# facebookresearch/KeypointNeRF

Measured on AMD Instinct MI355X. Metric: rendered rays/sec (64 coarse + 64 fine samples/ray), higher is better.
Workload: dtype f32 (dominant kernel: every fp32 operand as two fp16 pieces (22 bits, the residual formed exactly), three fp16-MFMA products per term set (hh hl lh: all terms above 2^-24 relative), fp32 accumulation; everything else fp32)

## Files before the change

include/kpnerf.h:

```cpp
#ifndef KPNERF_H
#define KPNERF_H

#include <stddef.h>
#include <stdint.h>

#ifdef __cplusplus
extern "C" {
#endif

#define KPN_ABI_VERSION 5
#define KPN_N_KPT 24
#define KPN_MAX_VIEWS 16

enum { KPN_OK = 0, KPN_EINVAL = -1, KPN_ELAUNCH = -2, KPN_EWORKSPACE = -3 };

int kpn_abi_version(void);
const char* kpn_last_error(void);
int kpn_is_device_build(void);

size_t kpn_plain_weight_floats(void);
size_t kpn_packed_weight_floats(void);
int kpn_pack_weights(const float* plain_host, float* packed_host);
int kpn_pack_weights_device(const float* plain_dev, float* packed_dev, void* stream);

typedef struct kpn_scene_desc {
    int32_t n_views;
    int32_t src_h, src_w;
    int32_t geo0_h, geo0_w;
    int32_t geo1_h, geo1_w;
    int32_t tex_h, tex_w;
    int32_t disable_fg_mask;
    float znear, zfar;
    float nml_scale;
    float sigma;
    const float* KRT;
    const float* extrin;
    const float* kpt3d;
    const float* img;
    const uint8_t* fg_mask;
    const float* geo0;
    const float* geo1;
    const float* tex;
} kpn_scene_desc;

size_t kpn_scene_workspace_bytes(const kpn_scene_desc* desc);
int kpn_scene_prepare(const kpn_scene_desc* desc, void* scene_ws, void* stream);


int kpn_ray_bbox_intersection(const float* bounds, const float* orig, const float* direct, int64_t n_rays,
                              float* near_out, float* far_out, uint8_t* hit_out, void* stream);

int kpn_make_rays(const float* K, const float* RT, float znear, float zfar, const float* bounds, int32_t x0,
                  int32_t y0, int32_t step, int32_t nx, int32_t ny, float* dirs, float* cam_pos, float* near_out,
                  float* far_out, void* stream);

int kpn_importance_sample(const float* contrib, const float* z, const float* u, int64_t n_rays, int32_t d_minus_2,
                          int32_t n_samples, float* samples_out, void* stream);

int kpn_rgba2out(const float* rgba, const float* z, int64_t n_rays, int32_t n_samples, float* color, float* depth,
                 float* alpha, float* contrib, float* sdf, void* stream);

int kpn_rgba2out_backward(const float* rgba, const float* z, int64_t n_rays, int32_t n_samples, const float* d_color,
                          const float* d_depth, const float* d_alpha, const float* d_sdf, float* d_rgba, void* stream);

size_t kpn_geo_rows_backward_workspace_bytes(int64_t n_points, int32_t n_views);
int kpn_geo_rows_backward(const kpn_scene_desc* desc, const void* scene_ws, const float* packed_weights, int64_t n_points,
                          const float* pts, uint32_t keep_mask, const float* d_x, float* d_plain, float* d_geo0,
                          float* d_geo1, void* workspace, size_t workspace_bytes, void* stream);

size_t kpn_query_backward_geometry_workspace_bytes(int64_t n_points, int32_t n_views);
int kpn_query_backward_geometry(const kpn_scene_desc* desc, const void* scene_ws, const float* packed_weights,
                                int64_t n_points, const float* pts, int32_t mode, uint32_t keep_mask, const float* noise,
                                float noise_std, const float* d_out, float* d_plain, float* d_geo0, float* d_geo1,
                                void* workspace, size_t workspace_bytes, void* stream);

size_t kpn_query_backward_workspace_bytes(int64_t n_points, int32_t n_views);
int kpn_query_backward(const kpn_scene_desc* desc, const void* scene_ws, const float* packed_weights, int64_t n_points,
                       const float* pts, const float* view, int32_t mode, uint32_t keep_mask, const float* noise,
                       float noise_std, const float* d_out, float* d_plain, float* d_geo0, float* d_geo1, float* d_tex,
                       void* workspace, size_t workspace_bytes, void* stream);

int kpn_set_geo_rows_mode(int32_t mode);
int kpn_get_geo_rows_mode(void);
int kpn_set_fuse_mode(int32_t mode);
int kpn_get_fuse_mode(void);
int kpn_set_density_first(int32_t mode);
int kpn_get_density_first(void);
int kpn_density_first_passes(int64_t* density_first, int64_t* fused, int32_t reset);
int kpn_density_stats(void* stream, int64_t* listed, int64_t* live, int32_t reset);
int kpn_packed_f16_range_check(const float* packed_weights_dev, void* stream, int32_t* beyond);
// ... 134 lines not shown
```

keypointnerf_amd/csrc/api_render.hip:

```cpp
namespace {
struct RenderLayout { size_t cam_pos, dirs, nearv, farv, zc, zf, zn, src, rgba, rgba_c, rgba_n, contrib, color, depth, alpha, sdf, query, total; int64_t chunk; };
int64_t pick_chunk(const kpn_scene_desc* d, const kpn_render_args* a) {
    const int64_t R = (int64_t)a->nx * a->ny;
    int64_t c = a->chunk_rays;
    if (c <= 0) {
        const int64_t cmax = 262144;
        const int64_t npass = (R + cmax - 1) / cmax;
        c = ((R + npass - 1) / npass + 63) / 64 * 64;
    }
    return c < R ? c : R;
}
RenderLayout render_layout(const kpn_scene_desc* d, const kpn_render_args* a) {
    RenderLayout L;
    const int64_t R = (int64_t)a->nx * a->ny;
    const int64_t C = pick_chunk(d, a);
    const int64_t Sfull = a->n_coarse + (a->fine ? a->n_fine : 0);
    Carver c;
    L.chunk = C;
    L.cam_pos = c.take(64);
    L.dirs = c.take((size_t)R * 3 * 4);
    L.nearv = c.take((size_t)R * 4);
    L.farv = c.take((size_t)R * 4);
    L.zc = c.take((size_t)C * a->n_coarse * 4);
    L.zf = c.take((size_t)C * Sfull * 4);
// ... 38 lines not shown
}

__global__ void k_store_planar(int64_t r0, int64_t n, int64_t R, int C, const float* __restrict__ src, float* __restrict__ dst) {
    const int64_t i = (int64_t)blockIdx.x * blockDim.x + threadIdx.x;
    if (i >= n * C) return;
    const int64_t r = i / C;
    const int c = (int)(i - r * C);
    dst[(int64_t)c * R + r0 + r] = src[i];
}
__global__ void k_load_planar(int64_t r0, int64_t n, int64_t R, int C, const float* __restrict__ src, float* __restrict__ dst) {
    const int64_t i = (int64_t)blockIdx.x * blockDim.x + threadIdx.x;
    if (i >= n * C) return;
    const int64_t r = i / C;
    const int c = (int)(i - r * C);
    dst[i] = src ? src[(int64_t)c * R + r0 + r] : 0.0f;
}
struct PlanarChunk {
    void* stream; int64_t r0, n, R;
    void store(float* dst, const float* src, int C) const {
        if (dst) KPN_LAUNCH(k_store_planar, grid1d(n * C, 256), dim3(256), stream, r0, n, R, C, src, dst);
    }
    void load(float* dst, const float* src, int C) const {
        KPN_LAUNCH(k_load_planar, grid1d(n * C, 256), dim3(256), stream, r0, n, R, C, src, dst);
    }
};

extern "C" size_t kpn_render_workspace_bytes(const kpn_scene_desc* d, const kpn_render_args* a) {
    if (check_desc(d) != KPN_OK || check_render(a) != KPN_OK) return 0;
    return render_layout(d, a).total;
}

static void launch_fine_samples(void* stream, int64_t n, int Sc, int Sf, const float* zc, const float* contrib,
                                const float* u, float* zf, float* znew, int16_t* src) {
    const dim3 grid((unsigned)(n + 3 < 4 * 8192 ? (n + 3) / 4 : 8192));
    if (Sc <= 64 && Sf <= 64)
        KPN_LAUNCH(k_fine_samples_w<true>, grid, dim3(256), stream, n, Sc, Sf, zc, contrib, u, zf, znew, src);
    else
        KPN_LAUNCH(k_fine_samples_w<false>, grid, dim3(256), stream, n, Sc, Sf, zc, contrib, u, zf, znew, src);
}

static int render_impl(const kpn_scene_desc* d, const void* scene_ws, const float* wp, const kpn_render_args* a,
                       const kpn_train_args* t, void* ws, size_t ws_bytes, void* stream) {
    if (int e = check_desc(d)) return e;
    if (int e = check_render(a)) return e;
    KPN_REQUIRE(scene_ws && wp && ws, "null pointer");
    if (t) if (int e = check_train(d, a, t, false)) return e;
    const RenderLayout L = render_layout(d, a);
    if (ws_bytes < L.total) return fail(KPN_EWORKSPACE, "render workspace too small");
    char* base = static_cast<char*>(ws);
    auto F = [&](size_t off) { return reinterpret_cast<float*>(base + off); };
    kpn_scene_dev sc = scene_dev(d, scene_ws);
    const int64_t R = (int64_t)a->nx * a->ny;
    const int Sc = a->n_coarse, Sf = a->fine ? a->n_fine : 0, Sfull = Sc + Sf;
    KPN_LAUNCH(k_make_rays, grid1d(R, 256), dim3(256), stream, a->K, a->RT, a->znear, a->zfar, a->bounds, (int)a->x0, (int)a->y0,
               (int)a->step, (int)(a->step_y > 0 ? a->step_y : a->step), (int)a->nx, (int)a->ny, t ? (const int*)t->pix : (const int*)nullptr, F(L.dirs), F(L.cam_pos),
               F(L.nearv), F(L.farv));
    for (int64_t r0 = 0; r0 < R; r0 += L.chunk) {
        const int64_t n = (R - r0) < L.chunk ? (R - r0) : L.chunk;
        const float* dirs = F(L.dirs) + r0 * 3;
        const PlanarChunk pl{stream, r0, n, R};
        KPN_LAUNCH(k_coarse_z, grid1d(n * Sc, 256), dim3(256), stream, n, Sc, (const float*)(F(L.nearv) + r0),
                   (const float*)(F(L.farv) + r0), t ? t->u_coarse + r0 * Sc : (const float*)nullptr, F(L.zc));
        kpn_points ps{nullptr, nullptr, F(L.cam_pos), dirs, F(L.zc), Sc,
                      (t && t->rand_noise_std != 0.0f) ? t->noise_coarse + r0 * Sc : nullptr, t ? t->rand_noise_std : 0.0f};
        sc.keep = t ? t->keep_coarse : 0xFFFFFFFFu;
        const char* nr = getenv("KPN_NO_COARSE_REUSE");
        const bool no_reuse = nr && atoi(nr);
        const bool reuse = (t == nullptr) && a->fine && !no_reuse;
        float* rgba_coarse = reuse ? F(L.rgba_c) : F(L.rgba);
        const int allow_pool = t == nullptr;
        if (int e = run_field(sc, ps, wp, n * Sc, 1, rgba_coarse, nullptr, base + L.query, stream, 1, 0, allow_pool, a->rows_kernel, a->fuse_kernel)) return e;
// ... 232 lines not shown
```

keypointnerf_amd/csrc/api_scene.hip:

```cpp
namespace {
struct SceneLayout { size_t table, rgbm, geo0, geo1, tex, flags, total; };
SceneLayout scene_layout(const kpn_scene_desc* d) {
    SceneLayout L;
    Carver c;
    L.table = c.take((size_t)d->n_views * KPN_TBL_STRIDE, 64);
    L.rgbm = c.take((size_t)d->n_views * d->src_h * d->src_w * 4, 64);
    L.geo0 = c.take((size_t)d->n_views * d->geo0_h * d->geo0_w * 64, 64);
    L.geo1 = c.take((size_t)d->n_views * d->geo1_h * d->geo1_w * 8, 64);
    L.tex = c.take((size_t)d->n_views * d->tex_h * d->tex_w * 8, 64);
    L.flags = c.take((size_t)KPN_SCENE_FLAG_FLOATS, 64);
    L.total = c.o;
    return L;
}
int check_desc(const kpn_scene_desc* d) {
    KPN_REQUIRE(d != nullptr, "scene desc is null");
    KPN_REQUIRE(d->n_views >= 1 && d->n_views <= KPN_MAX_VIEWS, "n_views out of range");
    KPN_REQUIRE(d->src_h > 1 && d->src_w > 1 && d->geo0_h > 1 && d->geo0_w > 1 && d->geo1_h > 1 && d->geo1_w > 1 &&
                d->tex_h > 1 && d->tex_w > 1, "map sizes must be > 1");
    KPN_REQUIRE(d->zfar > d->znear && d->nml_scale > 0.0f && d->sigma > 0.0f, "bad scalar parameters");
    KPN_REQUIRE(d->KRT && d->extrin && d->kpt3d && d->img && d->geo0 && d->geo1 && d->tex, "null scene tensor");
    KPN_REQUIRE(d->disable_fg_mask || d->fg_mask, "fg_mask is null");
    return KPN_OK;
}
kpn_scene_dev scene_dev(const kpn_scene_desc* d, const void* ws) {
    const SceneLayout L = scene_layout(d);
    const float* base = static_cast<const float*>(ws);
    kpn_scene_dev s;
    s.V = d->n_views; s.H = d->src_h; s.W = d->src_w;
    s.g0h = d->geo0_h; s.g0w = d->geo0_w; s.g1h = d->geo1_h; s.g1w = d->geo1_w; s.th = d->tex_h; s.tw = d->tex_w;
    s.disable_fg_mask = d->disable_fg_mask;
    s.znear = d->znear; s.zfar = d->zfar; s.nml_scale = d->nml_scale;
    s.two_sigma2 = (float)(2.0 * ((double)d->sigma * (double)d->sigma));
    s.keep = 0xFFFFFFFFu;
    s.table = base + L.table; s.rgbm = base + L.rgbm; s.geo0 = base + L.geo0; s.geo1 = base + L.geo1; s.tex = base + L.tex;
    s.flags = base + L.flags;
    return s;
}
}

extern "C" size_t kpn_scene_workspace_bytes(const kpn_scene_desc* d) {
    if (check_desc(d) != KPN_OK) return 0;
    return scene_layout(d).total * sizeof(float);
}

extern "C" int kpn_scene_prepare(const kpn_scene_desc* d, void* scene_ws, void* stream) {
    if (int e = check_desc(d)) return e;
    KPN_REQUIRE(scene_ws != nullptr, "scene workspace is null");
    const SceneLayout L = scene_layout(d);
    float* base = static_cast<float*>(scene_ws);
    const int V = d->n_views;
    float* flags = base + L.flags;
    KPN_LAUNCH(k_scene_table, dim3(1), dim3(64), stream, V, d->KRT, d->extrin, d->kpt3d, base + L.table, flags);
    const int64_t HW = (int64_t)d->src_h * d->src_w;
    KPN_LAUNCH(k_pack_rgbm, grid1d(V * HW, 256), dim3(256), stream, (int64_t)(V * HW), HW, d->img,
               d->disable_fg_mask ? (const uint8_t*)nullptr : d->fg_mask, base + L.rgbm, flags);
    const int64_t hw0 = (int64_t)d->geo0_h * d->geo0_w, hw1 = (int64_t)d->geo1_h * d->geo1_w, hwt = (int64_t)d->tex_h * d->tex_w;
    KPN_LAUNCH(k_nchw_to_nhwc, grid1d(V * hw0 * 64, 256), dim3(256), stream, (int64_t)(V * hw0 * 64), 64, hw0, d->geo0, base + L.geo0, flags);
    KPN_LAUNCH(k_nchw_to_nhwc, grid1d(V * hw1 * 8, 256), dim3(256), stream, (int64_t)(V * hw1 * 8), 8, hw1, d->geo1, base + L.geo1, flags);
    KPN_LAUNCH(k_nchw_to_nhwc, grid1d(V * hwt * 8, 256), dim3(256), stream, (int64_t)(V * hwt * 8), 8, hwt, d->tex, base + L.tex, flags);
    return check_launch("kpn_scene_prepare");
}

extern "C" int kpn_ray_bbox_intersection(const float* bounds, const float* orig, const float* direct, int64_t R,
                                         float* near_o, float* far_o, uint8_t* hit_o, void* stream) {
    KPN_REQUIRE(bounds && orig && direct && near_o && far_o && hit_o, "null pointer");
    KPN_REQUIRE(R >= 0, "negative ray count");
    if (R == 0) return KPN_OK;
    KPN_LAUNCH(k_ray_bbox, grid1d(R, 256), dim3(256), stream, R, bounds, orig, direct, near_o, far_o, hit_o);
    return check_launch("kpn_ray_bbox_intersection");
}

extern "C" int kpn_make_rays(const float* K, const float* RT, float znear, float zfar, const float* bounds, int32_t x0,
                             int32_t y0, int32_t step, int32_t nx, int32_t ny, float* dirs, float* cam_pos,
                             float* near_o, float* far_o, void* stream) {
    KPN_REQUIRE(K && RT && bounds && dirs && cam_pos && near_o && far_o, "null pointer");
    KPN_REQUIRE(nx > 0 && ny > 0 && step > 0, "bad pixel grid");
    KPN_LAUNCH(k_make_rays, grid1d((int64_t)nx * ny, 256), dim3(256), stream, K, RT, znear, zfar, bounds, (int)x0, (int)y0,
               (int)step, (int)step, (int)nx, (int)ny, (const int*)nullptr, dirs, cam_pos, near_o, far_o);
    return check_launch("kpn_make_rays");
}

extern "C" int kpn_importance_sample(const float* contrib, const float* z, const float* u, int64_t R, int32_t Dm2,
                                     int32_t n, float* out, void* stream) {
    KPN_REQUIRE(contrib && z && out, "null pointer");
    KPN_REQUIRE(Dm2 >= 1 && Dm2 + 1 <= KPN_IS_MAXD, "bin count out of range (<= 128)");
    KPN_REQUIRE(n >= 1 && R >= 0, "bad sizes");
    if (R == 0) return KPN_OK;
    KPN_LAUNCH(k_importance, grid1d(R, 64), dim3(64), stream, R, (int)Dm2, (int)n, contrib, z, u, out);
    return check_launch("kpn_importance_sample");
}

static void launch_rgba2out(void* stream, int64_t R, int S, const float* rgba, const float* z, float* color, float* depth,
// ... 39 lines not shown
```

keypointnerf_amd/csrc/ray_kernels.hip:

```cpp
#include "kpn_device.h"

__device__ __forceinline__ void kpn_note_absmax(float* __restrict__ flags, float a) {
    int u = __float_as_int(a) & 0x7fffffff;
#pragma unroll
    for (int o = 32; o > 0; o >>= 1) { const int w = __shfl_xor(u, o); u = w > u ? w : u; }
    int* f = reinterpret_cast<int*>(flags);
    if ((threadIdx.x & 63) == 0 && u > *reinterpret_cast<volatile int*>(f)) atomicMax(f, u);
}
__device__ __forceinline__ float kpn_absmax2(float a, float b) {
    const int x = __float_as_int(a) & 0x7fffffff, y = __float_as_int(b) & 0x7fffffff;
    return __int_as_float(x > y ? x : y);
}

__global__ void k_scene_table(int V, const float* __restrict__ KRT, const float* __restrict__ extrin,
                              const float* __restrict__ kpt3d, float* __restrict__ table, float* __restrict__ flags) {
    const int v = blockIdx.x * blockDim.x + threadIdx.x;
    if (v < KPN_SCENE_FLAG_FLOATS) flags[v] = 0.0f;
    if (v >= V) return;
    float* tb = table + (size_t)v * KPN_TBL_STRIDE;
    const float* M = KRT + v * 16;
    const float* E = extrin + v * 16;
    for (int i = 0; i < 12; ++i) { tb[KPN_TBL_KRT + i] = M[i]; tb[KPN_TBL_EXT + i] = E[i]; }
    double a[4][8];
    for (int i = 0; i < 4; ++i)
        for (int j = 0; j < 4; ++j) { a[i][j] = (double)M[i * 4 + j]; a[i][4 + j] = (i == j) ? 1.0 : 0.0; }
    for (int c = 0; c < 4; ++c) {
        int p = c;
        for (int r = c + 1; r < 4; ++r) if (fabs(a[r][c]) > fabs(a[p][c])) p = r;
        if (p != c) for (int j = 0; j < 8; ++j) { double t = a[c][j]; a[c][j] = a[p][j]; a[p][j] = t; }
        const double d = a[c][c];
        for (int j = 0; j < 8; ++j) a[c][j] /= d;
        for (int r = 0; r < 4; ++r) if (r != c) {
            const double f = a[r][c];
            for (int j = 0; j < 8; ++j) a[r][j] -= f * a[c][j];
        }
    }
    for (int i = 0; i < 3; ++i) tb[KPN_TBL_CPOS + i] = (float)a[i][7];
    tb[KPN_TBL_CPOS + 3] = 0.0f;
    for (int k = 0; k < KPN_NKPT; ++k)
        for (int i = 0; i < 3; ++i)
            tb[KPN_TBL_KCAM + k * 3 + i] =
                KADD(kpn_dot3(kpt3d[k * 3 + 0], kpt3d[k * 3 + 1], kpt3d[k * 3 + 2], E[i * 4 + 0], E[i * 4 + 1], E[i * 4 + 2]),
                     E[i * 4 + 3]);
    for (int i = KPN_TBL_KCAM + KPN_NKPT * 3; i < KPN_TBL_STRIDE; ++i) tb[i] = 0.0f;
}

__global__ void k_pack_rgbm(int64_t npix_total, int64_t HW, const float* __restrict__ img,
                            const uint8_t* __restrict__ mask, float* __restrict__ out, float* __restrict__ flags) {
    const int64_t i = (int64_t)blockIdx.x * blockDim.x + threadIdx.x;
    float amax = 0.0f;
    if (i < npix_total) {
        const int64_t v = i / HW, p = i - v * HW;
        float4 o;
        o.x = img[(v * 3 + 0) * HW + p];
        o.y = img[(v * 3 + 1) * HW + p];
        o.z = img[(v * 3 + 2) * HW + p];
        o.w = mask ? (mask[i] ? 1.0f : 0.0f) : 1.0f;
        reinterpret_cast<float4*>(out)[i] = o;
        amax = kpn_absmax2(kpn_absmax2(o.x, o.y), o.z);
    }
    kpn_note_absmax(flags, amax);
}

__global__ void k_nchw_to_nhwc(int64_t total, int C, int64_t hw, const float* __restrict__ in, float* __restrict__ out,
                               float* __restrict__ flags) {
    const int64_t i = (int64_t)blockIdx.x * blockDim.x + threadIdx.x;
    float x = 0.0f;
    if (i < total) {
        const int c = (int)(i % C);
        const int64_t vp = i / C;
        const int64_t v = vp / hw, p = vp - v * hw;
        x = in[(v * C + c) * hw + p];
        out[i] = x;
    }
    kpn_note_absmax(flags, x);
}

__device__ __forceinline__ void kpn_ray_aabb(const float* __restrict__ bounds, float ox, float oy, float oz, float dx,
                                             float dy, float dz, float& near_o, float& far_o, int& hit) {
    float bmin[3], bmax[3], o[3] = {ox, oy, oz}, d[3] = {dx, dy, dz};
#pragma unroll
    for (int i = 0; i < 3; ++i) {
        bmin[i] = KADD(bounds[i], -0.01f);
        bmax[i] = KADD(bounds[3 + i], 0.01f);
        if (fabsf(d[i]) < 1e-5f) d[i] = 1e-5f;
    }
    int cnt = 0;
    float pint[2][3];
    const float eps = 1e-6f;
#pragma unroll
    for (int s = 0; s < 6; ++s) {
        const int ax = s % 3;
        const float bound = (s < 3) ? bmin[ax] : bmax[ax];
        const float t = KSUB(bound, o[ax]) / d[ax];
        const float p0 = KADD(KMUL(t, d[0]), o[0]), p1 = KADD(KMUL(t, d[1]), o[1]), p2 = KADD(KMUL(t, d[2]), o[2]);
        const int inside = (p0 >= KSUB(bmin[0], eps)) && (p0 <= KADD(bmax[0], eps)) && (p1 >= KSUB(bmin[1], eps)) &&
                           (p1 <= KADD(bmax[1], eps)) && (p2 >= KSUB(bmin[2], eps)) && (p2 <= KADD(bmax[2], eps));
        if (inside) {
            if (cnt < 2) { pint[cnt][0] = p0; pint[cnt][1] = p1; pint[cnt][2] = p2; }
            ++cnt;
        }
    }
    if (cnt == 2) {
        const float nr = sqrtf(kpn_dot3(d[0], d[1], d[2], d[0], d[1], d[2]));
        float dd[2];
#pragma unroll
        for (int k = 0; k < 2; ++k) {
            const float e0 = KSUB(pint[k][0], o[0]), e1 = KSUB(pint[k][1], o[1]), e2 = KSUB(pint[k][2], o[2]);
// ... 292 lines not shown
                                                   const float* __restrict__ zin, const float* __restrict__ u,
                                                   float* __restrict__ out) {
    __shared__ float cdf_s[64][KPN_IS_MAXD];
    const int t = threadIdx.x;
    const int64_t r = (int64_t)blockIdx.x * 64 + t;
    if (r >= R) return;
    const int C = Dm2 + 1;
    const float* c = contrib + r * Dm2;
    const float* zz = zin + r * C;
    float sum = 0.0f;
    for (int i = 0; i < Dm2; ++i) sum = KADD(sum, KADD(c[i], 1e-5f));
    float run = 0.0f;
    cdf_s[t][0] = 0.0f;
    for (int i = 0; i < Dm2; ++i) {
        run = KADD(run, KADD(c[i], 1e-5f) / sum);
        cdf_s[t][i + 1] = run;
    }
    for (int k = 0; k < n; ++k) {
        const float s = u ? u[r * n + k] : kpn_linspace01(k, n);
        int lo = 0, hi = C;
        while (lo < hi) {
            const int mid = (lo + hi) >> 1;
            if (cdf_s[t][mid] <= s) lo = mid + 1; else hi = mid;
        }
        const int ip = lo - 1 < 0 ? 0 : lo - 1;
        const int in = lo > C - 1 ? C - 1 : lo;
        const float num = KSUB(s, cdf_s[t][ip]);
        float den = KSUB(cdf_s[t][in], cdf_s[t][ip]);
        if (den < 1e-5f) den = 1.0f;
        out[r * n + k] = KADD(zz[ip], KMUL(num / den, KSUB(zz[in], zz[ip])));
    }
}

#ifndef KPN_SIMT_EMU
#define KPN_READLANE_F(v, i) __int_as_float(__builtin_amdgcn_readlane(__float_as_int(v), (i)))
#else
#define KPN_READLANE_F(v, i) __shfl((v), (i))
#endif
template <bool SMALL>
__global__ __launch_bounds__(256) void k_fine_samples_w(int64_t R, int Sc, int Sf, const float* __restrict__ zc,
                                                        const float* __restrict__ contrib, const float* __restrict__ u,
                                                        float* __restrict__ zf, float* __restrict__ znew,
                                                        int16_t* __restrict__ src) {
    constexpr int NE = SMALL ? 1 : 2;
    constexpr int W = 64 * NE;
    __shared__ float q_s[SMALL ? 1 : 4][SMALL ? 1 : W];
    __shared__ float cdf_s[4][W + 1];
    __shared__ float zn_s[4][W];
    __shared__ float ev_s[4][2 * W];
    const int lane = threadIdx.x & 63, w = threadIdx.x >> 6;
    const int Dm2 = Sc - 2, C = Sc - 1, Sfull = Sc + Sf;
    for (int64_t r = (int64_t)blockIdx.x * 4 + w; r < R; r += (int64_t)gridDim.x * 4) {
        const float* c = contrib + r * Sc + 1;
        const float* z = zc + r * Sc;
        for (int i = lane; i < Sc; i += 64) ev_s[w][i] = z[i];
        if constexpr (SMALL) {
            float q = lane < Dm2 ? KADD(c[lane], 1e-5f) : 0.0f;
            float sum = 0.0f;
            for (int i = 0; i < Dm2; ++i) sum = KADD(sum, KPN_READLANE_F(q, i));
            q = q / sum;
            float run = 0.0f, mine = 0.0f;
            for (int i = 0; i < Dm2; ++i) {
                run = KADD(run, KPN_READLANE_F(q, i));
                mine = lane == i + 1 ? run : mine;
            }
            if (lane < C) cdf_s[w][lane] = mine;
        } else {
            for (int i = lane; i < Dm2; i += 64) q_s[w][i] = KADD(c[i], 1e-5f);
            KPN_WAVE_SYNC();
            float sum = 0.0f;
            if (lane == 0)
                for (int i = 0; i < Dm2; ++i) sum = KADD(sum, q_s[w][i]);
            sum = __shfl(sum, 0);
            for (int i = lane; i < Dm2; i += 64) q_s[w][i] = q_s[w][i] / sum;
            KPN_WAVE_SYNC();
            if (lane == 0) {
                float run = 0.0f;
                cdf_s[w][0] = 0.0f;
                for (int i = 0; i < Dm2; ++i) { run = KADD(run, q_s[w][i]); cdf_s[w][i + 1] = run; }
            }
        }
        KPN_WAVE_SYNC();
        float v[NE];
        for (int e = 0; e < NE; ++e) {
            const int k = lane + 64 * e;
            v[e] = 0.0f;
            if (k < Sf) {
                const float sv = u ? u[r * Sf + k] : kpn_linspace01(k, Sf);
                int lo = 0, hi = C;
                while (lo < hi) {
                    const int mid = (lo + hi) >> 1;
                    if (cdf_s[w][mid] <= sv) lo = mid + 1; else hi = mid;
                }
                const int ip = lo - 1 < 0 ? 0 : lo - 1;
                const int in = lo > C - 1 ? C - 1 : lo;
                const float num = KSUB(sv, cdf_s[w][ip]);
                float den = KSUB(cdf_s[w][in], cdf_s[w][ip]);
                if (den < 1e-5f) den = 1.0f;
                const float zp = KMUL(0.5f, KADD(ev_s[w][ip + 1], ev_s[w][ip]));
                const float zq = KMUL(0.5f, KADD(ev_s[w][in + 1], ev_s[w][in]));
                v[e] = KADD(zp, KMUL(num / den, KSUB(zq, zp)));
                zn_s[w][k] = v[e];
            }
        }
        KPN_WAVE_SYNC();
        int rk[NE];
        int unsorted = 0;
        for (int e = 0; e < NE; ++e) {
            const int k = lane + 64 * e;
            rk[e] = k;
            unsorted |= (k + 1 < Sf) && !(v[e] <= zn_s[w][k + 1 < W ? k + 1 : k]);
        }
        if (__any(unsorted)) {
            for (int e = 0; e < NE; ++e) rk[e] = 0;
            for (int j = 0; j < Sf; ++j) {
                const float o = zn_s[w][j];
                for (int e = 0; e < NE; ++e) rk[e] += (o < v[e]) || (o == v[e] && j < lane + 64 * e);
            }
        }
        for (int e = 0; e < NE; ++e)
            if (lane + 64 * e < Sf) ev_s[w][Sc + rk[e]] = v[e];
        KPN_WAVE_SYNC();
        if (znew)
            for (int k = lane; k < Sf; k += 64) znew[r * Sf + k] = ev_s[w][Sc + k];
        int csorted = 1;
        for (int i = lane; i + 1 < Sc; i += 64) csorted &= ev_s[w][i] <= ev_s[w][i + 1];
        if (__all(csorted)) {
            for (int i = lane; i < Sc; i += 64) {
                const float a = ev_s[w][i];
                int lo = 0, hi = Sf;
                while (lo < hi) { const int mid = (lo + hi) >> 1; if (ev_s[w][Sc + mid] < a) lo = mid + 1; else hi = mid; }
                zf[r * Sfull + i + lo] = a;
                if (src) src[r * Sfull + i + lo] = (int16_t)i;
            }
            for (int k = lane; k < Sf; k += 64) {
                const float b = ev_s[w][Sc + k];
                int lo = 0, hi = Sc;
                while (lo < hi) { const int mid = (lo + hi) >> 1; if (ev_s[w][mid] <= b) lo = mid + 1; else hi = mid; }
                zf[r * Sfull + k + lo] = b;
                if (src) src[r * Sfull + k + lo] = (int16_t)(Sc + k);
            }
        } else {
            for (int id = lane; id < Sfull; id += 64) {
                const float a = ev_s[w][id];
                int rank = 0;
                for (int j = 0; j < Sfull; ++j) { const float o = ev_s[w][j]; rank += (o < a) || (o == a && j < id); }
                zf[r * Sfull + rank] = a;
                if (src) src[r * Sfull + rank] = (int16_t)id;
            }
        }
        KPN_WAVE_SYNC();
    }
}

__global__ void k_frame_to_rgb8(int HW, int bgr, const float* __restrict__ chw, uint8_t* __restrict__ hwc) {
    const int i = blockIdx.x * blockDim.x + threadIdx.x;
    if (i >= HW) return;
#pragma unroll
    for (int c = 0; c < 3; ++c) {
        const float v = fminf(fmaxf(chw[(size_t)c * HW + i], 0.0f), 1.0f);
        hwc[(size_t)i * 3 + (bgr ? 2 - c : c)] = (uint8_t)(int)KMUL(v, 255.0f);
    }
}

__global__ __launch_bounds__(256) void k_mse_psnr(int64_t n, const float* __restrict__ a, const float* __restrict__ b,
                                                  double* __restrict__ partial, int* __restrict__ ticket,
                                                  double* __restrict__ out2) {
    __shared__ double red[256];
    __shared__ int last;
    double acc = 0.0;
    for (int64_t i = (int64_t)blockIdx.x * blockDim.x + threadIdx.x; i < n; i += (int64_t)gridDim.x * blockDim.x) {
        const float d = KSUB(a[i], b[i]);
        acc += (double)KMUL(d, d);
    }
    red[threadIdx.x] = acc;
    __syncthreads();
    for (int s = 128; s > 0; s >>= 1) {
        if ((int)threadIdx.x < s) red[threadIdx.x] += red[threadIdx.x + s];
        __syncthreads();
    }
    if (threadIdx.x == 0) {
        partial[blockIdx.x] = red[0];
        __threadfence();
        last = (atomicAdd(ticket, 1) == (int)gridDim.x - 1);
// ... 107 lines not shown
```

keypointnerf_amd/lib.py:

```python
import ctypes
import os

import torch

_HERE = os.path.dirname(os.path.abspath(__file__))
DEFAULT_LIB = os.path.join(_HERE, "_lib", "libkpnerf_hip.so")

c_f = ctypes.c_float
c_i32 = ctypes.c_int32
c_i64 = ctypes.c_int64
c_p = ctypes.c_void_p
c_sz = ctypes.c_size_t


class SceneDesc(ctypes.Structure):
    _fields_ = [(n, c_i32) for n in ("n_views", "src_h", "src_w", "geo0_h", "geo0_w", "geo1_h", "geo1_w", "tex_h",
                                     "tex_w", "disable_fg_mask")] + \
               [(n, c_f) for n in ("znear", "zfar", "nml_scale", "sigma")] + \
               [(n, c_p) for n in ("KRT", "extrin", "kpt3d", "img", "fg_mask", "geo0", "geo1", "tex")]


class RenderStages(ctypes.Structure):
    _fields_ = [(n, c_p) for n in ("z_coarse", "rgba_coarse", "z_fine", "rgba_fine", "dirs", "cam_pos")]


class RenderArgs(ctypes.Structure):
    _fields_ = [(n, c_p) for n in ("K", "RT", "bounds")] + [("znear", c_f), ("zfar", c_f)] + \
               [(n, c_i32) for n in ("x0", "y0", "step", "nx", "ny", "n_coarse", "n_fine", "fine", "chunk_rays")] + \
               [(n, c_p) for n in ("tex_fg", "depth", "alpha", "tex_fg_fine", "depth_fine", "alpha_fine", "sdf")] + \
               [("step_y", c_i32), ("rows_kernel", c_i32), ("fuse_kernel", c_i32), ("stages", ctypes.POINTER(RenderStages))]


class TrainArgs(ctypes.Structure):
    _fields_ = [(n, c_p) for n in ("pix", "u_coarse", "noise_coarse", "noise_fine", "u_fine")] + \
               [("keep_coarse", ctypes.c_uint32), ("keep_fine", ctypes.c_uint32), ("rand_noise_std", c_f)]


class RenderGrads(ctypes.Structure):
    _fields_ = [(n, c_p) for n in ("d_tex_fg", "d_depth", "d_alpha", "d_tex_fg_fine", "d_depth_fine", "d_alpha_fine", "d_sdf")]


_SIGNATURES = {
    "kpn_abi_version": (ctypes.c_int, []),
    "kpn_last_error": (ctypes.c_char_p, []),
    "kpn_is_device_build": (ctypes.c_int, []),
    "kpn_plain_weight_floats": (c_sz, []),
    "kpn_packed_weight_floats": (c_sz, []),
    "kpn_pack_weights": (ctypes.c_int, [c_p, c_p]),
    "kpn_pack_weights_device": (ctypes.c_int, [c_p, c_p, c_p]),
    "kpn_scene_workspace_bytes": (c_sz, [ctypes.POINTER(SceneDesc)]),
    "kpn_scene_prepare": (ctypes.c_int, [ctypes.POINTER(SceneDesc), c_p, c_p]),
    "kpn_ray_bbox_intersection": (ctypes.c_int, [c_p, c_p, c_p, c_i64, c_p, c_p, c_p, c_p]),
    "kpn_make_rays": (ctypes.c_int, [c_p, c_p, c_f, c_f, c_p, c_i32, c_i32, c_i32, c_i32, c_i32, c_p, c_p, c_p, c_p, c_p]),
    "kpn_importance_sample": (ctypes.c_int, [c_p, c_p, c_p, c_i64, c_i32, c_i32, c_p, c_p]),
    "kpn_rgba2out": (ctypes.c_int, [c_p, c_p, c_i64, c_i32, c_p, c_p, c_p, c_p, c_p, c_p]),
    "kpn_rgba2out_backward": (ctypes.c_int, [c_p, c_p, c_i64, c_i32, c_p, c_p, c_p, c_p, c_p, c_p]),
    "kpn_geo_rows_backward_workspace_bytes": (c_sz, [c_i64, c_i32]),
    "kpn_geo_rows_backward": (ctypes.c_int, [ctypes.POINTER(SceneDesc), c_p, c_p, c_i64, c_p, ctypes.c_uint32, c_p, c_p, c_p,
                                             c_p, c_p, c_sz, c_p]),
    "kpn_query_backward_geometry_workspace_bytes": (c_sz, [c_i64, c_i32]),
    "kpn_query_backward_geometry": (ctypes.c_int, [ctypes.POINTER(SceneDesc), c_p, c_p, c_i64, c_p, c_i32, ctypes.c_uint32, c_p,
                                                   ctypes.c_float, c_p, c_p, c_p, c_p, c_p, c_sz, c_p]),
    "kpn_query_backward_workspace_bytes": (c_sz, [c_i64, c_i32]),
    "kpn_query_backward": (ctypes.c_int, [ctypes.POINTER(SceneDesc), c_p, c_p, c_i64, c_p, c_p, c_i32, ctypes.c_uint32, c_p,
                                          ctypes.c_float, c_p, c_p, c_p, c_p, c_p, c_p, c_sz, c_p]),
    "kpn_render_rays_train_backward_workspace_bytes": (c_sz, [ctypes.POINTER(SceneDesc), ctypes.POINTER(RenderArgs)]),
    "kpn_render_rays_train_backward": (ctypes.c_int, [ctypes.POINTER(SceneDesc), c_p, c_p, ctypes.POINTER(RenderArgs),
                                                      ctypes.POINTER(TrainArgs), ctypes.POINTER(RenderGrads), c_p, c_p, c_p, c_p,
                                                      c_p, c_sz, c_p]),
    "kpn_set_geo_rows_mode": (ctypes.c_int, [c_i32]),
    "kpn_get_geo_rows_mode": (ctypes.c_int, []),
    "kpn_packed_f16_range_check": (ctypes.c_int, [c_p, c_p, c_p]),
    "kpn_set_fuse_mode": (ctypes.c_int, [c_i32]),
    "kpn_get_fuse_mode": (ctypes.c_int, []),
    "kpn_set_density_first": (ctypes.c_int, [c_i32]),
    "kpn_get_density_first": (ctypes.c_int, []),
    "kpn_density_stats": (ctypes.c_int, [c_p, c_p, c_p, c_i32]),
    "kpn_density_first_passes": (ctypes.c_int, [c_p, c_p, c_i32]),
    "kpn_bwd_profile_enable": (ctypes.c_int, [c_i32]),
    "kpn_bwd_profile_collect": (ctypes.c_int, [c_p, c_p, c_p, c_p, c_p]),
    "kpn_set_range_guard": (ctypes.c_int, [c_i32]),
    "kpn_get_range_guard": (ctypes.c_int, []),
    "kpn_range_guard_count": (ctypes.c_int, [c_p, c_p]),
    "kpn_ssim_scratch_bytes": (c_sz, [c_i32, c_i32]),
    "kpn_ssim": (ctypes.c_int, [c_p, c_p, c_i32, c_i32, c_i32, c_i32, c_i32, c_i32, c_p, c_p, c_p]),
    "kpn_query_workspace_bytes": (c_sz, [c_i64, c_i32]),
    "kpn_query": (ctypes.c_int, [ctypes.POINTER(SceneDesc), c_p, c_p, c_i64, c_p, c_p, c_i32, c_p, c_p, c_p, c_sz, c_p]),
# ... 87 lines not shown
```

Before: 12.79 million.

## Batch fine-sample CDF builds per thread and grid-stride scene copy kernels

The fine-sampling kernel now processes a block of 128 (or 64) rays at once. It stages contributions in shared memory and has one thread per ray compute the normalized CDF, replacing the per-wave readlane serial prefix. Scene-prepare copy kernels become grid-stride loops with a capped grid, and their absmax flag update is reduced per block before a single atomic. A standalone kpn_fine_samples entry point is also exported. The changes add block-wide barriers and more shared memory use, and the per-thread serial CDF loop may leave lanes idle.

After: 13.12 million (median of 6 runs). +2.6%, better.

```diff
diff --git a/include/kpnerf.h b/include/kpnerf.h
--- a/include/kpnerf.h
+++ b/include/kpnerf.h
@@ -56,6 +56,9 @@
 
 int kpn_importance_sample(const float* contrib, const float* z, const float* u, int64_t n_rays, int32_t d_minus_2,
                           int32_t n_samples, float* samples_out, void* stream);
+
+int kpn_fine_samples(const float* z_coarse, const float* contrib, const float* u, int64_t n_rays, int32_t n_coarse,
+                     int32_t n_fine, float* z_fine, float* z_new, int16_t* src, void* stream);
 
 int kpn_rgba2out(const float* rgba, const float* z, int64_t n_rays, int32_t n_samples, float* color, float* depth,
                  float* alpha, float* contrib, float* sdf, void* stream);
diff --git a/keypointnerf_amd/csrc/api_render.hip b/keypointnerf_amd/csrc/api_render.hip
--- a/keypointnerf_amd/csrc/api_render.hip
+++ b/keypointnerf_amd/csrc/api_render.hip
@@ -94,11 +94,27 @@
 
 static void launch_fine_samples(void* stream, int64_t n, int Sc, int Sf, const float* zc, const float* contrib,
                                 const float* u, float* zf, float* znew, int16_t* src) {
-    const dim3 grid((unsigned)(n + 3 < 4 * 8192 ? (n + 3) / 4 : 8192));
-    if (Sc <= 64 && Sf <= 64)
+    const bool small = Sc <= 64 && Sf <= 64;
+    const int64_t rb = small ? 128 : 64;
+    const int64_t groups = (n + rb - 1) / rb;
+#ifndef KPN_SIMT_EMU
+    const int64_t max_groups = 8192;
+#else
+    const int64_t max_groups = 2;
+#endif
+    const dim3 grid((unsigned)(groups < max_groups ? groups : max_groups));
+    if (small)
         KPN_LAUNCH(k_fine_samples_w<true>, grid, dim3(256), stream, n, Sc, Sf, zc, contrib, u, zf, znew, src);
     else
         KPN_LAUNCH(k_fine_samples_w<false>, grid, dim3(256), stream, n, Sc, Sf, zc, contrib, u, zf, znew, src);
+}
+extern "C" int kpn_fine_samples(const float* z_coarse, const float* contrib, const float* u, int64_t n_rays, int32_t n_coarse,
+                                int32_t n_fine, float* z_fine, float* z_new, int16_t* src, void* stream) {
+    KPN_REQUIRE(n_rays >= 0 && n_coarse >= 3 && n_coarse <= 128 && n_fine >= 1 && n_fine <= 128, "sample counts must be 3..128 coarse, 1..128 fine");
+    if (n_rays == 0) return KPN_OK;
+    KPN_REQUIRE(z_coarse && contrib && z_fine, "null pointer");
+    launch_fine_samples(stream, n_rays, n_coarse, n_fine, z_coarse, contrib, u, z_fine, z_new, src);
+    return check_launch("kpn_fine_samples");
 }
 
 static int render_impl(const kpn_scene_desc* d, const void* scene_ws, const float* wp, const kpn_render_args* a,
diff --git a/keypointnerf_amd/csrc/api_scene.hip b/keypointnerf_amd/csrc/api_scene.hip
--- a/keypointnerf_amd/csrc/api_scene.hip
+++ b/keypointnerf_amd/csrc/api_scene.hip
@@ -51,13 +51,19 @@
     const int V = d->n_views;
     float* flags = base + L.flags;
     KPN_LAUNCH(k_scene_table, dim3(1), dim3(64), stream, V, d->KRT, d->extrin, d->kpt3d, base + L.table, flags);
+#ifndef KPN_SIMT_EMU
+    const int64_t kCopyGroups = 2048;
+#else
+    const int64_t kCopyGroups = 2;
+#endif
+    auto copy_grid = [&](int64_t n) { const int64_t g = (n + 255) / 256; return dim3((unsigned)(g < kCopyGroups ? g : kCopyGroups)); };
     const int64_t HW = (int64_t)d->src_h * d->src_w;
-    KPN_LAUNCH(k_pack_rgbm, grid1d(V * HW, 256), dim3(256), stream, (int64_t)(V * HW), HW, d->img,
+    KPN_LAUNCH(k_pack_rgbm, copy_grid(V * HW), dim3(256), stream, (int64_t)(V * HW), HW, d->img,
                d->disable_fg_mask ? (const uint8_t*)nullptr : d->fg_mask, base + L.rgbm, flags);
     const int64_t hw0 = (int64_t)d->geo0_h * d->geo0_w, hw1 = (int64_t)d->geo1_h * d->geo1_w, hwt = (int64_t)d->tex_h * d->tex_w;
-    KPN_LAUNCH(k_nchw_to_nhwc, grid1d(V * hw0 * 64, 256), dim3(256), stream, (int64_t)(V * hw0 * 64), 64, hw0, d->geo0, base + L.geo0, flags);
-    KPN_LAUNCH(k_nchw_to_nhwc, grid1d(V * hw1 * 8, 256), dim3(256), stream, (int64_t)(V * hw1 * 8), 8, hw1, d->geo1, base + L.geo1, flags);
-    KPN_LAUNCH(k_nchw_to_nhwc, grid1d(V * hwt * 8, 256), dim3(256), stream, (int64_t)(V * hwt * 8), 8, hwt, d->tex, base + L.tex, flags);
+    KPN_LAUNCH(k_nchw_to_nhwc, copy_grid(V * hw0 * 64), dim3(256), stream, (int64_t)(V * hw0 * 64), 64, hw0, d->geo0, base + L.geo0, flags);
+    KPN_LAUNCH(k_nchw_to_nhwc, copy_grid(V * hw1 * 8), dim3(256), stream, (int64_t)(V * hw1 * 8), 8, hw1, d->geo1, base + L.geo1, flags);
+    KPN_LAUNCH(k_nchw_to_nhwc, copy_grid(V * hwt * 8), dim3(256), stream, (int64_t)(V * hwt * 8), 8, hwt, d->tex, base + L.tex, flags);
     return check_launch("kpn_scene_prepare");
 }
 
diff --git a/keypointnerf_amd/csrc/ray_kernels.hip b/keypointnerf_amd/csrc/ray_kernels.hip
--- a/keypointnerf_amd/csrc/ray_kernels.hip
+++ b/keypointnerf_amd/csrc/ray_kernels.hip
@@ -1,11 +1,17 @@
 #include "kpn_device.h"
 
-__device__ __forceinline__ void kpn_note_absmax(float* __restrict__ flags, float a) {
+__device__ __forceinline__ void kpn_note_absmax(float* __restrict__ flags, float a, int* wave_max ) {
     int u = __float_as_int(a) & 0x7fffffff;
 #pragma unroll
     for (int o = 32; o > 0; o >>= 1) { const int w = __shfl_xor(u, o); u = w > u ? w : u; }
-    int* f = reinterpret_cast<int*>(flags);
-    if ((threadIdx.x & 63) == 0 && u > *reinterpret_cast<volatile int*>(f)) atomicMax(f, u);
+    if ((threadIdx.x & 63) == 0) wave_max[(threadIdx.x >> 6) & 3] = u;
+    __syncthreads();
+    if (threadIdx.x == 0) {
+        const int nw = (int)((blockDim.x + 63) >> 6);
+        for (int k = 1; k < nw && k < 4; ++k) u = wave_max[k] > u ? wave_max[k] : u;
+        int* f = reinterpret_cast<int*>(flags);
+        if (u > *reinterpret_cast<volatile int*>(f)) atomicMax(f, u);
+    }
 }
 __device__ __forceinline__ float kpn_absmax2(float a, float b) {
     const int x = __float_as_int(a) & 0x7fffffff, y = __float_as_int(b) & 0x7fffffff;
@@ -45,11 +51,11 @@
     for (int i = KPN_TBL_KCAM + KPN_NKPT * 3; i < KPN_TBL_STRIDE; ++i) tb[i] = 0.0f;
 }
 
-__global__ void k_pack_rgbm(int64_t npix_total, int64_t HW, const float* __restrict__ img,
-                            const uint8_t* __restrict__ mask, float* __restrict__ out, float* __restrict__ flags) {
-    const int64_t i = (int64_t)blockIdx.x * blockDim.x + threadIdx.x;
+__global__ __launch_bounds__(256) void k_pack_rgbm(int64_t npix_total, int64_t HW, const float* __restrict__ img,
+                                                   const uint8_t* __restrict__ mask, float* __restrict__ out, float* __restrict__ flags) {
+    __shared__ int wave_max[4];
     float amax = 0.0f;
-    if (i < npix_total) {
+    for (int64_t i = (int64_t)blockIdx.x * blockDim.x + threadIdx.x; i < npix_total; i += (int64_t)gridDim.x * blockDim.x) {
         const int64_t v = i / HW, p = i - v * HW;
         float4 o;
         o.x = img[(v * 3 + 0) * HW + p];
@@ -57,23 +63,24 @@
         o.z = img[(v * 3 + 2) * HW + p];
         o.w = mask ? (mask[i] ? 1.0f : 0.0f) : 1.0f;
         reinterpret_cast<float4*>(out)[i] = o;
-        amax = kpn_absmax2(kpn_absmax2(o.x, o.y), o.z);
-    }
-    kpn_note_absmax(flags, amax);
-}
-
-__global__ void k_nchw_to_nhwc(int64_t total, int C, int64_t hw, const float* __restrict__ in, float* __restrict__ out,
-                               float* __restrict__ flags) {
-    const int64_t i = (int64_t)blockIdx.x * blockDim.x + threadIdx.x;
-    float x = 0.0f;
-    if (i < total) {
+        amax = kpn_absmax2(amax, kpn_absmax2(kpn_absmax2(o.x, o.y), o.z));
+    }
+    kpn_note_absmax(flags, amax, wave_max);
+}
+
+__global__ __launch_bounds__(256) void k_nchw_to_nhwc(int64_t total, int C, int64_t hw, const float* __restrict__ in, float* __restrict__ out,
+                                                      float* __restrict__ flags) {
+    __shared__ int wave_max[4];
+    float amax = 0.0f;
+    for (int64_t i = (int64_t)blockIdx.x * blockDim.x + threadIdx.x; i < total; i += (int64_t)gridDim.x * blockDim.x) {
         const int c = (int)(i % C);
         const int64_t vp = i / C;
         const int64_t v = vp / hw, p = vp - v * hw;
-        x = in[(v * C + c) * hw + p];
+        const float x = in[(v * C + c) * hw + p];
         out[i] = x;
-    }
-    kpn_note_absmax(flags, x);
+        amax = kpn_absmax2(amax, x);
+    }
+    kpn_note_absmax(flags, amax, wave_max);
 }
 
 __device__ __forceinline__ void kpn_ray_aabb(const float* __restrict__ bounds, float ox, float oy, float oz, float dx,
@@ -432,11 +439,6 @@
     }
 }
 
-#ifndef KPN_SIMT_EMU
-#define KPN_READLANE_F(v, i) __int_as_float(__builtin_amdgcn_readlane(__float_as_int(v), (i)))
-#else
-#define KPN_READLANE_F(v, i) __shfl((v), (i))
-#endif
 template <bool SMALL>
 __global__ __launch_bounds__(256) void k_fine_samples_w(int64_t R, int Sc, int Sf, const float* __restrict__ zc,
                                                         const float* __restrict__ contrib, const float* __restrict__ u,
@@ -444,112 +446,111 @@
                                                         int16_t* __restrict__ src) {
     constexpr int NE = SMALL ? 1 : 2;
     constexpr int W = 64 * NE;
-    __shared__ float q_s[SMALL ? 1 : 4][SMALL ? 1 : W];
-    __shared__ float cdf_s[4][W + 1];
+    constexpr int RB = SMALL ? 128 : 64;
+    constexpr int CS = W - 1;
+    __shared__ float cdf_s[RB * CS];
     __shared__ float zn_s[4][W];
     __shared__ float ev_s[4][2 * W];
     const int lane = threadIdx.x & 63, w = threadIdx.x >> 6;
     const int Dm2 = Sc - 2, C = Sc - 1, Sfull = Sc + Sf;
-    for (int64_t r = (int64_t)blockIdx.x * 4 + w; r < R; r += (int64_t)gridDim.x * 4) {
-        const float* c = contrib + r * Sc + 1;
-        const float* z = zc + r * Sc;
-        for (int i = lane; i < Sc; i += 64) ev_s[w][i] = z[i];
-        if constexpr (SMALL) {
-            float q = lane < Dm2 ? KADD(c[lane], 1e-5f) : 0.0f;
+    for (int64_t g0 = (int64_t)blockIdx.x * RB; g0 < R; g0 += (int64_t)gridDim.x * RB) {
+        const int nr = (int)(R - g0 < RB ? R - g0 : RB);
+        for (int row = w; row < nr; row += 4) {
+            const float* c = contrib + (g0 + row) * Sc + 1;
+            for (int i = lane; i < Dm2; i += 64) cdf_s[row * CS + i] = KADD(c[i], 1e-5f);
+        }
+        __syncthreads();
+        if ((int)threadIdx.x < nr && C > 0) {
+            float* q = cdf_s + (int)threadIdx.x * CS;
             float sum = 0.0f;
-            for (int i = 0; i < Dm2; ++i) sum = KADD(sum, KPN_READLANE_F(q, i));
-            q = q / sum;
-            float run = 0.0f, mine = 0.0f;
+            for (int i = 0; i < Dm2; ++i) sum = KADD(sum, q[i]);
+            float run = 0.0f, nxt = Dm2 > 0 ? q[0] : 0.0f;
+            q[0] = 0.0f;
             for (int i = 0; i < Dm2; ++i) {
-                run = KADD(run, KPN_READLANE_F(q, i));
-                mine = lane == i + 1 ? run : mine;
-            }
-            if (lane < C) cdf_s[w][lane] = mine;
-        } else {
-            for (int i = lane; i < Dm2; i += 64) q_s[w][i] = KADD(c[i], 1e-5f);
+                const float cur = nxt;
+                if (i + 1 < Dm2) nxt = q[i + 1];
+                run = KADD(run, cur / sum);
+                q[i + 1] = run;
+            }
+        }
+        __syncthreads();
+        for (int row = w; row < nr; row += 4) {
+            const int64_t r = g0 + row;
+            const float* cdf = cdf_s + row * CS;
+            const float* z = zc + r * Sc;
+            for (int i = lane; i < Sc; i += 64) ev_s[w][i] = z[i];
             KPN_WAVE_SYNC();
-            float sum = 0.0f;
-            if (lane == 0)
-                for (int i = 0; i < Dm2; ++i) sum = KADD(sum, q_s[w][i]);
-            sum = __shfl(sum, 0);
-            for (int i = lane; i < Dm2; i += 64) q_s[w][i] = q_s[w][i] / sum;
+            float v[NE];
+            for (int e = 0; e < NE; ++e) {
+                const int k = lane + 64 * e;
+                v[e] = 0.0f;
+                if (k < Sf) {
+                    const float sv = u ? u[r * Sf + k] : kpn_linspace01(k, Sf);
+                    int lo = 0, hi = C;
+                    while (lo < hi) {
+                        const int mid = (lo + hi) >> 1;
+                        if (cdf[mid] <= sv) lo = mid + 1; else hi = mid;
+                    }
+                    const int ip = lo - 1 < 0 ? 0 : lo - 1;
+                    const int in = lo > C - 1 ? C - 1 : lo;
+                    const float num = KSUB(sv, cdf[ip]);
+                    float den = KSUB(cdf[in], cdf[ip]);
+                    if (den < 1e-5f) den = 1.0f;
+                    const float zp = KMUL(0.5f, KADD(ev_s[w][ip + 1], ev_s[w][ip]));
+                    const float zq = KMUL(0.5f, KADD(ev_s[w][in + 1], ev_s[w][in]));
+                    v[e] = KADD(zp, KMUL(num / den, KSUB(zq, zp)));
+                    zn_s[w][k] = v[e];
+                }
+            }
             KPN_WAVE_SYNC();
-            if (lane == 0) {
-                float run = 0.0f;
-                cdf_s[w][0] = 0.0f;
-                for (int i = 0; i < Dm2; ++i) { run = KADD(run, q_s[w][i]); cdf_s[w][i + 1] = run; }
-            }
-        }
-        KPN_WAVE_SYNC();
-        float v[NE];
-        for (int e = 0; e < NE; ++e) {
-            const int k = lane + 64 * e;
-            v[e] = 0.0f;
-            if (k < Sf) {
-                const float sv = u ? u[r * Sf + k] : kpn_linspace01(k, Sf);
-                int lo = 0, hi = C;
-                while (lo < hi) {
-                    const int mid = (lo + hi) >> 1;
-                    if (cdf_s[w][mid] <= sv) lo = mid + 1; else hi = mid;
+            int rk[NE];
+            int unsorted = 0;
+            for (int e = 0; e < NE; ++e) {
+                const int k = lane + 64 * e;
+                rk[e] = k;
+                unsorted |= (k + 1 < Sf) && !(v[e] <= zn_s[w][k + 1 < W ? k + 1 : k]);
+            }
+            if (__any(unsorted)) {
+                for (int e = 0; e < NE; ++e) rk[e] = 0;
+                for (int j = 0; j < Sf; ++j) {
+                    const float o = zn_s[w][j];
+                    for (int e = 0; e < NE; ++e) rk[e] += (o < v[e]) || (o == v[e] && j < lane + 64 * e);
                 }
-                const int ip = lo - 1 < 0 ? 0 : lo - 1;
-                const int in = lo > C - 1 ? C - 1 : lo;
-                const float num = KSUB(sv, cdf_s[w][ip]);
-                float den = KSUB(cdf_s[w][in], cdf_s[w][ip]);
-                if (den < 1e-5f) den = 1.0f;
-                const float zp = KMUL(0.5f, KADD(ev_s[w][ip + 1], ev_s[w][ip]));
-                const float zq = KMUL(0.5f, KADD(ev_s[w][in + 1], ev_s[w][in]));
-                v[e] = KADD(zp, KMUL(num / den, KSUB(zq, zp)));
-                zn_s[w][k] = v[e];
-            }
-        }
-        KPN_WAVE_SYNC();
-        int rk[NE];
-        int unsorted = 0;
-        for (int e = 0; e < NE; ++e) {
-            const int k = lane + 64 * e;
-            rk[e] = k;
-            unsorted |= (k + 1 < Sf) && !(v[e] <= zn_s[w][k + 1 < W ? k + 1 : k]);
-        }
-        if (__any(unsorted)) {
-            for (int e = 0; e < NE; ++e) rk[e] = 0;
-            for (int j = 0; j < Sf; ++j) {
-                const float o = zn_s[w][j];
-                for (int e = 0; e < NE; ++e) rk[e] += (o < v[e]) || (o == v[e] && j < lane + 64 * e);
-            }
-        }
-        for (int e = 0; e < NE; ++e)
-            if (lane + 64 * e < Sf) ev_s[w][Sc + rk[e]] = v[e];
-        KPN_WAVE_SYNC();
-        if (znew)
-            for (int k = lane; k < Sf; k += 64) znew[r * Sf + k] = ev_s[w][Sc + k];
-        int csorted = 1;
-        for (int i = lane; i + 1 < Sc; i += 64) csorted &= ev_s[w][i] <= ev_s[w][i + 1];
-        if (__all(csorted)) {
-            for (int i = lane; i < Sc; i += 64) {
-                const float a = ev_s[w][i];
-                int lo = 0, hi = Sf;
-                while (lo < hi) { const int mid = (lo + hi) >> 1; if (ev_s[w][Sc + mid] < a) lo = mid + 1; else hi = mid; }
-                zf[r * Sfull + i + lo] = a;
-                if (src) src[r * Sfull + i + lo] = (int16_t)i;
-            }
-            for (int k = lane; k < Sf; k += 64) {
-                const float b = ev_s[w][Sc + k];
-                int lo = 0, hi = Sc;
-                while (lo < hi) { const int mid = (lo + hi) >> 1; if (ev_s[w][mid] <= b) lo = mid + 1; else hi = mid; }
-                zf[r * Sfull + k + lo] = b;
-                if (src) src[r * Sfull + k + lo] = (int16_t)(Sc + k);
-            }
-        } else {
-            for (int id = lane; id < Sfull; id += 64) {
-                const float a = ev_s[w][id];
-                int rank = 0;
-                for (int j = 0; j < Sfull; ++j) { const float o = ev_s[w][j]; rank += (o < a) || (o == a && j < id); }
-                zf[r * Sfull + rank] = a;
-                if (src) src[r * Sfull + rank] = (int16_t)id;
-            }
-        }
-        KPN_WAVE_SYNC();
+            }
+            for (int e = 0; e < NE; ++e)
+                if (lane + 64 * e < Sf) ev_s[w][Sc + rk[e]] = v[e];
+            KPN_WAVE_SYNC();
+            if (znew)
+                for (int k = lane; k < Sf; k += 64) znew[r * Sf + k] = ev_s[w][Sc + k];
+            int csorted = 1;
+            for (int i = lane; i + 1 < Sc; i += 64) csorted &= ev_s[w][i] <= ev_s[w][i + 1];
+            if (__all(csorted)) {
+                for (int i = lane; i < Sc; i += 64) {
+                    const float a = ev_s[w][i];
+                    int lo = 0, hi = Sf;
+                    while (lo < hi) { const int mid = (lo + hi) >> 1; if (ev_s[w][Sc + mid] < a) lo = mid + 1; else hi = mid; }
+                    zf[r * Sfull + i + lo] = a;
+                    if (src) src[r * Sfull + i + lo] = (int16_t)i;
+                }
+                for (int k = lane; k < Sf; k += 64) {
+                    const float b = ev_s[w][Sc + k];
+                    int lo = 0, hi = Sc;
+                    while (lo < hi) { const int mid = (lo + hi) >> 1; if (ev_s[w][mid] <= b) lo = mid + 1; else hi = mid; }
+                    zf[r * Sfull + k + lo] = b;
+                    if (src) src[r * Sfull + k + lo] = (int16_t)(Sc + k);
+                }
+            } else {
+                for (int id = lane; id < Sfull; id += 64) {
+                    const float a = ev_s[w][id];
+                    int rank = 0;
+                    for (int j = 0; j < Sfull; ++j) { const float o = ev_s[w][j]; rank += (o < a) || (o == a && j < id); }
+                    zf[r * Sfull + rank] = a;
+                    if (src) src[r * Sfull + rank] = (int16_t)id;
+                }
+            }
+            KPN_WAVE_SYNC();
+        }
+        __syncthreads();
     }
 }
 
diff --git a/keypointnerf_amd/lib.py b/keypointnerf_amd/lib.py
--- a/keypointnerf_amd/lib.py
+++ b/keypointnerf_amd/lib.py
@@ -53,6 +53,7 @@
     "kpn_ray_bbox_intersection": (ctypes.c_int, [c_p, c_p, c_p, c_i64, c_p, c_p, c_p, c_p]),
     "kpn_make_rays": (ctypes.c_int, [c_p, c_p, c_f, c_f, c_p, c_i32, c_i32, c_i32, c_i32, c_i32, c_p, c_p, c_p, c_p, c_p]),
     "kpn_importance_sample": (ctypes.c_int, [c_p, c_p, c_p, c_i64, c_i32, c_i32, c_p, c_p]),
+    "kpn_fine_samples": (ctypes.c_int, [c_p, c_p, c_p, c_i64, c_i32, c_i32, c_p, c_p, c_p, c_p]),
     "kpn_rgba2out": (ctypes.c_int, [c_p, c_p, c_i64, c_i32, c_p, c_p, c_p, c_p, c_p, c_p]),
     "kpn_rgba2out_backward": (ctypes.c_int, [c_p, c_p, c_i64, c_i32, c_p, c_p, c_p, c_p, c_p, c_p]),
     "kpn_geo_rows_backward_workspace_bytes": (c_sz, [c_i64, c_i32]),
```
